# facebookresearch/pytorch3d

Measured on NVIDIA H100. Metric: rasterize frames/sec (fwd+bwd) 512^2 K=8, higher is better.
Workload: dtype f32

## Files before the change

pytorch3d_b200/csrc/binning.cuh:

```cuda
#pragma once
#include <climits>

#include "common.cuh"
#include "raster_math.cuh"

namespace b200r {

constexpr uint32_t RECT_EMPTY_X = 0x0000FFFFu;

__device__ __forceinline__ void pixel_range(float vmin, float vmax, int S, float range, int& lo, int& hi) {
  const float off = range * 0.5f, scale = (float)S / range, margin = 1e-3f + 1e-6f * (float)S;
  float a = (vmin + off) * scale - 0.5f - margin;
  float b = (vmax + off) * scale - 0.5f + margin;
  a = fminf(fmaxf(a, -1.0f), (float)S + 1.0f);
  b = fminf(fmaxf(b, -2.0f), (float)S);
  lo = max(0, (int)ceilf(a));
  hi = min(S - 1, (int)floorf(b));
}

__device__ __forceinline__ uint2 bbox_to_tile_rect(float xmin, float xmax, float ymin, float ymax, int H, int W,
                                                   float rx, float ry) {
  int ix_lo, ix_hi, iy_lo, iy_hi;
  pixel_range(xmin, xmax, W, rx, ix_lo, ix_hi);
  pixel_range(ymin, ymax, H, ry, iy_lo, iy_hi);
// ... 9 lines not shown
  const int64_t i = ((int64_t)blockIdx.x * 256 + threadIdx.x) * 4;
  pdl_trigger();
  if (i + 4 <= n && (reinterpret_cast<uintptr_t>(p) & 15u) == 0)
    *reinterpret_cast<int4*>(p + i) = make_int4(0, 0, 0, 0);
  else
    for (int64_t j = i; j < n && j < i + 4; ++j) p[j] = 0;
}

template <bool AGG = true>
__device__ __forceinline__ void warp_count_rect(uint2 r, int n, int TY, int TX, int* __restrict__ tile_count,
                                                int lane) {
  const bool empty = rect_empty(r);
  const int tx0 = r.x & 0xFFFF, tx1 = r.x >> 16, ty0 = r.y & 0xFFFF, ty1 = r.y >> 16;
  if (!AGG) {
    if (empty) return;
    for (int ty = ty0; ty <= ty1; ++ty)
      for (int tx = tx0; tx <= tx1; ++tx) atomicAdd(tile_count + (n * TY + ty) * TX + tx, 1);
    return;
  }
  const int w = empty ? 1 : tx1 - tx0 + 1;
  const int ntile = empty ? 0 : w * (ty1 - ty0 + 1);
  const int rounds = (int)__reduce_max_sync(0xffffffffu, (unsigned)ntile);
  int tx = tx0, ty = ty0;
  for (int i = 0; i < rounds; ++i) {
    const bool act = i < ntile;
    const int t = act ? (n * TY + ty) * TX + tx : -1 - lane;
    const int tprev = __shfl_up_sync(0xffffffffu, t, 1);
    const bool cont = act && lane > 0 && t == tprev;
    const unsigned conts = __ballot_sync(0xffffffffu, cont);
    if (act && !cont) {
      const unsigned after = lane == 31 ? 0u : conts >> (lane + 1);
      atomicAdd(tile_count + t, 1 + (__ffs((int)~after) - 1));
    }
    if (++tx > tx1) {
      tx = tx0;
      ++ty;
    }
  }
}

constexpr int ORDER_BITS = 21, ORDER_CLASSES = 3;
__device__ __forceinline__ int order_class(int count, int mean) { return count <= 0 ? 2 : (count > mean ? 0 : 1); }
__device__ __forceinline__ unsigned long long order_key(int count, int mean) {
  return 1ull << (ORDER_BITS * order_class(count, mean));
}

static __global__ void __launch_bounds__(1024) tile_scan_kernel(int* __restrict__ counts, int* __restrict__ offsets, int n,
                                                                int* __restrict__ order) {
  __shared__ long long warp_sums[32];
  __shared__ long long carry_s;
  __shared__ unsigned long long order_sums[32];
  __shared__ unsigned long long order_total, order_carry;
  __shared__ int nonempty_s;
  const int tid = threadIdx.x, lane = tid & 31, wid = tid >> 5;
  if (tid == 0) {
    carry_s = 0;
    nonempty_s = 0;
  }
  pdl_trigger();
  pdl_wait();
  __syncthreads();
  for (int base = 0; base < n; base += 8192) {
    const int i0 = base + tid * 8;
    int v[8];
    const bool vec = i0 + 8 <= n && ((reinterpret_cast<uintptr_t>(counts) | reinterpret_cast<uintptr_t>(offsets)) & 15u) == 0;
    if (vec) {
// ... 318 lines not shown
      } else {
        buf[phase * NT + i] = key;
        __syncthreads();
        other = buf[phase * NT + (i ^ d)];
        phase ^= 1;
      }
      B200R_CE64(other, (i & d) == 0);
    }
  }
#undef B200R_CE64
  return key;
}

template <int NT = TILE_THREADS>
__device__ __forceinline__ void cta_sort_segment(int* seg, int n, int* s_keys, int cap) {
  const bool in_smem = n <= cap;
  int* keys = in_smem ? s_keys : seg;
  if (in_smem)
    for (int i = threadIdx.x; i < n; i += NT) s_keys[i] = seg[i];
  __syncthreads();
  for (int k = 2; (k >> 1) < n; k <<= 1) {
    sort_sweep<true, NT>(keys, n, k);
    __syncthreads();
    for (int d = k >> 2; d > 0; d >>= 1) {
      sort_sweep<false, NT>(keys, n, d);
      __syncthreads();
    }
  }
  if (in_smem)
    for (int i = threadIdx.x; i < n; i += NT) seg[i] = s_keys[i];
  __syncthreads();
}

struct BinWorkspace {
  int* tile_count;
  int* tile_offset;
  int* tile_order;
  uint4* rect;
  int* pairs;
  int64_t capacity;
  size_t bytes;
};

inline int64_t default_pair_capacity(int64_t E, int N, int H, int W, int tile_h = TILE, int tile_w = TILE) {
  const int64_t tiles = (int64_t)div_up(H, tile_h) * div_up(W, tile_w);
  const int64_t exact = E * tiles;
  const int64_t heur = 32 * E + 64 * (int64_t)N * tiles;
  int64_t c = exact < heur ? exact : heur;
  if (c < 16) c = 16;
  if (c > 0x7fffffff) c = 0x7fffffff;
  return c;
}

inline BinWorkspace carve_workspace(void* base, int64_t E, int N, int H, int W, int64_t capacity, int tile_h = TILE,
                                    int tile_w = TILE) {
  BinWorkspace ws;
  const int64_t ntiles = (int64_t)N * div_up(H, tile_h) * div_up(W, tile_w);
  if (capacity <= 0) capacity = default_pair_capacity(E, N, H, W, tile_h, tile_w);
  ws.capacity = capacity;
  size_t off = 0;
  char* p = static_cast<char*>(base);
  ws.tile_count = reinterpret_cast<int*>(p + off);
  off = align_up(off + sizeof(int) * (size_t)ntiles, 16);
  ws.tile_offset = reinterpret_cast<int*>(p + off);
  off = align_up(off + sizeof(int) * (size_t)(ntiles + 1), 16);
  ws.tile_order = reinterpret_cast<int*>(p + off);
  off = align_up(off + sizeof(int) * (size_t)ntiles, 16);
  ws.rect = reinterpret_cast<uint4*>(p + off);
  off = align_up(off + sizeof(uint4) * (size_t)(E > 0 ? E : 1), 16);
  ws.pairs = reinterpret_cast<int*>(p + off);
  off = align_up(off + sizeof(int) * (size_t)capacity, 16);
  ws.bytes = off;
  return ws;
}

__device__ __forceinline__ unsigned box_pixel_mask(const float4 bx, const float (&col)[8], const float (&row)[4]) {
  unsigned xm = 0, ym = 0;
#pragma unroll
  for (int c = 0; c < 8; ++c) xm |= (!(col[c] > bx.y || col[c] < bx.x) ? 1u : 0u) << c;
#pragma unroll
  for (int r = 0; r < 4; ++r) ym |= (!(row[r] > bx.w || row[r] < bx.z) ? 1u : 0u) << (8 * r);
  return xm * ym;
}

__device__ __forceinline__ unsigned warp_transpose_bits(unsigned a, int lane) {
#pragma unroll
  for (int sft = 16; sft >= 1; sft >>= 1) {
    const unsigned lo = sft == 16 ? 0x0000FFFFu
                      : sft == 8 ? 0x00FF00FFu
                      : sft == 4 ? 0x0F0F0F0Fu
                      : sft == 2 ? 0x33333333u : 0x55555555u;
    const unsigned other = __shfl_xor_sync(0xffffffffu, a, sft);
    a = (lane & sft) ? ((a & ~lo) | ((other & ~lo) >> sft)) : ((a & lo) | ((other & lo) << sft));
  }
  return a;
}

}
```

pytorch3d_b200/csrc/raster_meshes.cu:

```cuda
#include <cfloat>
#include <climits>
#include <numeric>

#include "binning.cuh"
#include "bulk_copy.cuh"
#include "common.cuh"
#include "raster_math.cuh"

namespace b200r {

constexpr int SETUP_FACES = 256;
#ifndef B200R_MESH_TILE_H
#define B200R_MESH_TILE_H 16
#endif
constexpr int FTW = 16, FTH = B200R_MESH_TILE_H, FTHREADS = FTW * FTH;
static_assert(FTH == 16 || FTH == 8, "16x16 or 16x8 tiles");
constexpr int CHUNK = FTHREADS;
constexpr int SMEMQ_MAX_K = 32;

__device__ __forceinline__ bool face_is_drawable(const Face& f, bool cull_backfaces) {
  const float zmax = fmaxf(fmaxf(f.z0, f.z1), f.z2), zmin = fminf(fminf(f.z0, f.z1), f.z2);
  if (!(zmax >= 0.0f)) return false;
  if ((double)zmin < kEps) return false;
  const float area = edge_fn(f.x0, f.y0, f.x1, f.y1, f.x2, f.y2);
// ... 10 lines not shown
  ymax = fadd(fmaxf(fmaxf(f.y0, f.y1), f.y2), sqrt_blur);
}

constexpr size_t FACE_RECORD_BYTES = 4 * 16;

__device__ __forceinline__ void exact_pixel_range(float vmin, float vmax, int S, float range, int& lo, int& hi) {
  const float off = range * 0.5f, scale = (float)S / range, margin = 1e-3f + 1e-6f * (float)S;
  const float a = (vmin + off) * scale - 0.5f, b = (vmax + off) * scale - 0.5f;
  const float a0 = fminf(fmaxf(a - margin, -1.0f), (float)S + 1.0f), a1 = fminf(fmaxf(a + margin, -1.0f), (float)S + 1.0f);
  const float b0 = fminf(fmaxf(b + margin, -2.0f), (float)S), b1 = fminf(fmaxf(b - margin, -2.0f), (float)S);
  lo = max(0, (int)ceilf(a0));
  hi = min(S - 1, (int)floorf(b0));
  const bool lo_sure = lo == max(0, (int)ceilf(a1)) && a == a;
  const bool hi_sure = hi == min(S - 1, (int)floorf(b1)) && b == b;
  if (!lo_sure) {
    while (lo <= hi) {
      const float v = pix_to_ndc(lo, S, range);
      if (!(v > vmax || v < vmin)) break;
      ++lo;
    }
  }
  if (!hi_sure) {
    while (hi >= lo) {
      const float v = pix_to_ndc(hi, S, range);
      if (!(v > vmax || v < vmin)) break;
      --hi;
    }
  }
}

#ifndef B200R_SETUP_CTAS
#define B200R_SETUP_CTAS 1
#endif
template <bool INDEXED>
__global__ void __launch_bounds__(SETUP_FACES, B200R_SETUP_CTAS)
    mesh_setup_count_kernel(const float* __restrict__ face_verts, const float* __restrict__ verts, int64_t V,
                            const int64_t* __restrict__ faces, float* __restrict__ face_verts_out,
                            const int64_t* __restrict__ neighbor, int64_t F, const int64_t* __restrict__ first,
                            const int64_t* __restrict__ num, int N, int H, int W, int TY, int TX, float rx, float ry,
                            float sqrt_blur, int cull_backfaces, uint4* __restrict__ rect,
                            int* __restrict__ tile_count, float4* __restrict__ rec) {
  __shared__ __align__(16) float s_fv[SETUP_FACES * 9];
  __shared__ __align__(8) uint64_t bar;
  const int tid = threadIdx.x;
  const int64_t f0 = (int64_t)blockIdx.x * SETUP_FACES;
  const int nf = (int)min((int64_t)SETUP_FACES, F - f0);
  pdl_trigger();
  if (INDEXED) {
    for (int e = tid; e < nf * 3; e += SETUP_FACES) {
      const int64_t vi = __ldg(faces + f0 * 3 + e);
      const bool ok = vi >= 0 && vi < V;
      const float* v = verts + vi * 3;
      s_fv[e * 3 + 0] = ok ? __ldg(v + 0) : __int_as_float(0x7fc00000);
      s_fv[e * 3 + 1] = ok ? __ldg(v + 1) : __int_as_float(0x7fc00000);
      s_fv[e * 3 + 2] = ok ? __ldg(v + 2) : __int_as_float(0x7fc00000);
    }
    __syncthreads();
    for (int e = tid; e < nf * 9; e += SETUP_FACES) face_verts_out[f0 * 9 + e] = s_fv[e];
  } else {
    if (tid == 0) {
      mbar_init(&bar, 1);
      fence_mbar_init();
    }
    __syncthreads();
    cta_load_words(s_fv, face_verts + f0 * 9, nf * 9, &bar, 0);
  }
  uint2 r = make_uint2(RECT_EMPTY_X, 0u);
  int n = -1;
  const int64_t fi = f0 + tid;
  if (tid < nf) {
    const float* v = s_fv + tid * 9;
    const Face f = {v[0], v[1], v[2], v[3], v[4], v[5], v[6], v[7], v[8]};
    n = find_owner(first, num, N, fi);
    float4 box = make_float4(FLT_MAX, -FLT_MAX, FLT_MAX, -FLT_MAX);
    int4 rng = make_int4(1, 0, 1, 0);
    if (n >= 0 && face_is_drawable(f, cull_backfaces != 0)) {
      face_box(f, sqrt_blur, box.x, box.y, box.z, box.w);
      int ix_lo, ix_hi, iy_lo, iy_hi;
      exact_pixel_range(box.x, box.y, W, rx, ix_lo, ix_hi);
      exact_pixel_range(box.z, box.w, H, ry, iy_lo, iy_hi);
      if (ix_lo <= ix_hi && iy_lo <= iy_hi) {
        rng = make_int4(W - 1 - ix_hi, W - 1 - ix_lo, H - 1 - iy_hi, H - 1 - iy_lo);
        r = make_uint2((uint32_t)(rng.x / FTW) | ((uint32_t)(rng.y / FTW) << 16),
                       (uint32_t)(rng.z / FTH) | ((uint32_t)(rng.w / FTH) << 16));
      }
    }
    rect[fi] = make_uint4(r.x, r.y, (uint32_t)max(n, 0), 0u);
    const int nb = neighbor ? (int)__ldg(neighbor + fi) : -1;
    float4* out = rec + fi * 4;
    out[0] = make_float4(f.x0, f.y0, f.x1, f.y1);
    out[1] = make_float4(f.x2, f.y2, bary_denominator(f), __int_as_float((int)fi));
    out[2] = make_float4(f.z0, f.z1, f.z2, __int_as_float(nb));
    out[3] = sqrt_blur > 0.0f ? box
                              : make_float4(__int_as_float(rng.x), __int_as_float(rng.y), __int_as_float(rng.z),
                                            __int_as_float(rng.w));
  }
  pdl_wait();
  warp_count_rect(r, n, TY, TX, tile_count, tid & 31);
}

struct Hit {
  float z, dist, b0, b1, b2;
};

__device__ __forceinline__ void flag_tie();

template <bool WATCH>
__device__ __forceinline__ bool eval_pixel_face(float px, float py, const Face& f, float den, float blur_radius,
                                                bool persp, bool clip, bool full, float max_z, Hit& h) {
  const float e0 = edge_fn(px, py, f.x1, f.y1, f.x2, f.y2);
  const float e1 = edge_fn(px, py, f.x2, f.y2, f.x0, f.y0);
  const float e2 = edge_fn(px, py, f.x0, f.y0, f.x1, f.y1);
  float w0 = fdiv(e0, den), w1 = fdiv(e1, den), w2 = fdiv(e2, den);
  if (persp) bary_persp(w0, w1, w2, f.z0, f.z1, f.z2);
  float c0 = w0, c1 = w1, c2 = w2;
  if (clip) bary_clip(c0, c1, c2);
  const float pz = ffma(f.z2, c2, ffma(f.z0, c0, fmul(f.z1, c1)));
  if (!(pz >= 0.0f)) return false;
  if (full && !(pz < max_z)) {
    if (WATCH && pz == max_z) flag_tie();
    return false;
  }
  const bool inside = w0 > 0.0f && w1 > 0.0f && w2 > 0.0f;
  if (!inside && !(blur_radius > 0.0f)) return false;
  const float dist = point_tri_dist(px, py, f);
  if (!inside && dist >= blur_radius) return false;
  h.z = pz;
  h.dist = inside ? -dist : dist;
  h.b0 = c0;
  h.b1 = c1;
  h.b2 = c2;
// ... 205 lines not shown
};

__device__ __forceinline__ void stage_face(FaceChunk& s, int slot, const float* __restrict__ face_verts,
                                           const int64_t* __restrict__ neighbor, int f, float sqrt_blur,
                                           bool cull_backfaces) {
  const float* v = face_verts + (int64_t)f * 9;
  const Face fc = {__ldg(v + 0), __ldg(v + 1), __ldg(v + 2), __ldg(v + 3), __ldg(v + 4),
                   __ldg(v + 5), __ldg(v + 6), __ldg(v + 7), __ldg(v + 8)};
  float xmin = FLT_MAX, xmax = -FLT_MAX, ymin = FLT_MAX, ymax = -FLT_MAX;
  if (face_is_drawable(fc, cull_backfaces)) face_box(fc, sqrt_blur, xmin, xmax, ymin, ymax);
  s.box[slot] = make_float4(xmin, xmax, ymin, ymax);
  s.a[slot] = make_float4(fc.x0, fc.y0, fc.x1, fc.y1);
  s.b[slot] = make_float4(fc.x2, fc.y2, bary_denominator(fc), __int_as_float(f));
  const int nb = neighbor ? (int)__ldg(neighbor + f) : -1;
  s.c[slot] = make_float4(fc.z0, fc.z1, fc.z2, __int_as_float(nb));
}

template <typename T>
__device__ __forceinline__ void out_store(T* ptr, const T v) {
  __stcs(ptr, v);
}

struct FineParams {
  const float* face_verts;
  const int64_t* neighbor;
  const float4* rec;
  const int64_t* first;
  const int64_t* num;
  const int* tile_offset;
  const int* tile_order;
  int row_stride;
  int* pairs;
  int64_t capacity;
  int n0;
  int N, H, W, K, TY, TX;
  float rx, ry, blur_radius, sqrt_blur;
  int persp, clip, cull;
  int smem_ints;
  int64_t* pix_to_face;
  float* zbuf;
  float* bary;
  float* dists;
};

__device__ __forceinline__ void thread_pixel(int tile_x, int tile_y, int& xo, int& yo) {
  const int lane = threadIdx.x & 31, w = threadIdx.x >> 5;
  xo = tile_x * TILE + (w & 1) * 8 + (lane & 7);
  yo = tile_y * TILE + (w >> 1) * 4 + (lane >> 3);
}
__device__ __forceinline__ void fthread_pixel(int tile_x, int tile_y, int& xo, int& yo) {
  const int lane = threadIdx.x & 31, w = threadIdx.x >> 5;
  xo = tile_x * FTW + (w & 1) * 8 + (lane & 7);
  yo = tile_y * FTH + (w >> 1) * 4 + (lane >> 3);
}

__device__ __forceinline__ float warp_min(float v) {
#pragma unroll
  for (int d = 16; d > 0; d >>= 1) v = fminf(v, __shfl_xor_sync(0xffffffffu, v, d));
  return v;
}
__device__ __forceinline__ float warp_max(float v) {
#pragma unroll
  for (int d = 16; d > 0; d >>= 1) v = fmaxf(v, __shfl_xor_sync(0xffffffffu, v, d));
  return v;
}

// ... 138 lines not shown
  if (NB && nb != -1 && q.offer_neighbor(h, fi, nb)) return;
  q.offer(h, fi);
}

__device__ __forceinline__ float face_depth_lower_bound(const float4 fa, const float4 fb, const float4 fc, float cx,
                                                        float cy, float hx, float hy, bool persp, bool clip) {
  const float z0 = fc.x, z1 = fc.y, z2 = fc.z;
  if (clip) return fminf(fminf(z0, z1), z2) * (1.0f - 1e-6f);
  if (persp) return -FLT_MAX;
  const float x0 = fa.x, y0 = fa.y, x1 = fa.z, y1 = fa.w, x2 = fb.x, y2 = fb.y;
  const float rd = 1.0f / fabsf(fb.z);
  const float e0 = (cx - x1) * (y2 - y1) - (cy - y1) * (x2 - x1);
  const float e1 = (cx - x2) * (y0 - y2) - (cy - y2) * (x0 - x2);
  const float e2 = (cx - x0) * (y1 - y0) - (cy - y0) * (x1 - x0);
  const float num = z0 * e0 + z1 * e1 + z2 * e2;
  const float gxn = z0 * (y2 - y1) + z1 * (y0 - y2) + z2 * (y1 - y0);
  const float gyn = z0 * (x2 - x1) + z1 * (x0 - x2) + z2 * (x1 - x0);
  const float pzc = (fb.z < 0.0f ? -num : num) * rd;
  const float spread = (fabsf(gxn) * hx + fabsf(gyn) * hy) * rd;
  const float dx = fmaxf(fmaxf(fabsf(cx - x0), fabsf(cx - x1)), fabsf(cx - x2)) + hx;
  const float dy = fmaxf(fmaxf(fabsf(cy - y0), fabsf(cy - y1)), fabsf(cy - y2)) + hy;
  const float lx = fmaxf(fmaxf(x0, x1), x2) - fminf(fminf(x0, x1), x2);
  const float ly = fmaxf(fmaxf(y0, y1), y2) - fminf(fminf(y0, y1), y2);
  const float zabs = fmaxf(fmaxf(fabsf(z0), fabsf(z1)), fabsf(z2));
  const float margin = 1e-5f * (zabs * (dx * ly + dy * lx) * rd + fabsf(pzc) + spread);
  const float lb = pzc - spread - margin;
  return lb == lb ? lb : -FLT_MAX;
}

enum { ORDER_ARRIVAL = 0, ORDER_INDEX = 1 };

template <class Q, bool NB, bool SCAN>
__device__ __forceinline__ void fine_tile_body(const FineParams& p, FineStage& sh, Q& q, int tile_x, int tile_y, int n,
                                               int seg_begin, int count, bool overflow, int order, bool valid, int lc,
                                               int lr) {
  const int tid = threadIdx.x, lane = tid & 31;
  const bool persp = p.persp != 0, clip = p.clip != 0;
  const float blur_radius = p.blur_radius;
  const bool sorted_walk = order == ORDER_INDEX;
  const bool sort_staged = sorted_walk && !overflow && count <= CHUNK;
  if (sorted_walk && !overflow && count > CHUNK)
    cta_sort_segment<FTHREADS>(p.pairs + seg_begin, count, reinterpret_cast<int*>(&sh), p.smem_ints);
  if (tid < FTW + FTH) {
    if (tid < FTW)
      sh.col[tid] = pix_to_ndc(p.W - 1 - (tile_x * FTW + tid), p.W, p.rx);
    else
      sh.row[tid - FTW] = pix_to_ndc(p.H - 1 - (tile_y * FTH + tid - FTW), p.H, p.ry);
  }
  if (!sorted_walk && tid == FTW + FTH) sh.tie = 0;

  for (int base = 0; base < count; base += CHUNK) {
    const int nc = min(CHUNK, count - base);
    const int nwords = (nc + 31) >> 5;
    if (base > 0) __syncthreads();
    int f = INT_MAX;
    if (tid < nc) f = overflow ? (int)(p.first[n] + base + tid) : p.pairs[seg_begin + base + tid];
    if (sort_staged) {
      f = cta_sort256<FTHREADS>(f, nc, sh.u.sort_buf);
      if (nc > 32) __syncthreads();
    }
    if (tid < nc) {
      const float4* r = p.rec + (int64_t)f * 4;
      const float4 ra = __ldg(r + 0), rb = __ldg(r + 1), rc = __ldg(r + 2), rd = __ldg(r + 3);
      sh.a[tid] = ra;
      sh.b[tid] = rb;
      sh.c[tid] = rc;
      if (SCAN) {
        const int gx = __float_as_int(rd.x), gy = __float_as_int(rd.y), gz = __float_as_int(rd.z),
                  gw = __float_as_int(rd.w);
        const int c_lo = max(gx - tile_x * FTW, 0), c_hi = min(gy - tile_x * FTW, FTW - 1);
        const int r_lo = max(gz - tile_y * FTH, 0), r_hi = min(gw - tile_y * FTH, FTH - 1);
        sh.rng[tid] = (c_lo > c_hi || r_lo > r_hi) ? 1u
                                                   : (unsigned)(c_lo | (c_hi << 8) | (r_lo << 16) | (r_hi << 24));
      } else {
        sh.u.box[tid] = rd;
      }
    }
    if (SCAN) {
      for (int w = 0; w < nwords; ++w) sh.u.mask[w][tid] = 0u;
    }
    __syncthreads();
    if (SCAN) {
#ifndef B200R_SCAN_LANES
#define B200R_SCAN_LANES 4
#endif
      constexpr int SL = B200R_SCAN_LANES;
      const int dr = tid & (SL - 1);
      for (int fslot = tid / SL; fslot < nc; fslot += FTHREADS / SL) {
        const unsigned rg = sh.rng[fslot];
// ... 83 lines not shown
            __all_sync(0xffffffffu, !keep1 || (cmin >= b1.x && cmax <= b1.y && rmin >= b1.z && rmax <= b1.w));
        if (all0 && all1) {
          m0 = __ballot_sync(0xffffffffu, keep0);
          m1 = __ballot_sync(0xffffffffu, keep1);
        } else {
          float col[8], row[4];
#pragma unroll
          for (int c = 0; c < 8; ++c) col[c] = sh.col[(lc & 8) + c];
#pragma unroll
          for (int r = 0; r < 4; ++r) row[r] = sh.row[(lr & 12) + r];
          if (keep0) m0 = box_pixel_mask(b0, col, row);
          if (keep1) m1 = box_pixel_mask(b1, col, row);
          m0 = warp_transpose_bits(m0, lane);
          if (sub + 32 < nc) m1 = warp_transpose_bits(m1, lane);
        }
      }
      unsigned long long mine = valid ? (((unsigned long long)m1 << 32) | m0) : 0ull;
      while (__any_sync(0xffffffffu, mine != 0ull)) {
        if (mine != 0ull) {
          const int j = sub + __ffsll((long long)mine) - 1;
          mine &= mine - 1ull;
          consider_face<Q, NB>(sh, j, px, py, blur_radius, persp, clip, q);
        }
      }
    }
  }
}

__device__ __forceinline__ bool tile_saw_tie(const FineStage& sh) {
  return __syncthreads_or(sh.tie) != 0;
}

struct TileWork {
  int tile_x, tile_y, n, seg_begin, count;
  bool overflow;
};
__device__ __forceinline__ TileWork tile_work(const FineParams& p) {
  pdl_wait();
  TileWork t;
  int i;
  if (p.tile_order != nullptr) {
    i = p.tile_order[((p.n0 + blockIdx.z) * p.TY + blockIdx.y) * p.TX + blockIdx.x];
    t.tile_x = i % p.TX;
    const int r = i / p.TX;
    t.tile_y = r % p.TY;
    t.n = r / p.TY;
  } else {
    t.tile_x = blockIdx.x;
    t.tile_y = (int)((blockIdx.y * (unsigned)p.row_stride) % (unsigned)p.TY);
    t.n = p.n0 + blockIdx.z;
    i = (t.n * p.TY + t.tile_y) * p.TX + t.tile_x;
  }
  t.seg_begin = p.tile_offset[i];
  const int seg_end = p.tile_offset[i + 1];
  t.overflow = (int64_t)seg_end > p.capacity || seg_end == INT_MAX;
  t.count = t.overflow ? (int)p.num[t.n] : seg_end - t.seg_begin;
  return t;
}

template <bool NB, bool SCAN>
__device__ __forceinline__ int first_walk_order(const TileWork& t) {
  if (t.overflow || NB) return ORDER_INDEX;
  if (SCAN) return ORDER_ARRIVAL;
  return ORDER_INDEX;
}

#ifndef B200R_FINE_CTAS
#define B200R_FINE_CTAS 4
#endif
#ifndef B200R_FINE_SCAN_CTAS
#define B200R_FINE_SCAN_CTAS 3
#endif
#ifndef B200R_SMEMQ_CTAS
#define B200R_SMEMQ_CTAS 3
#endif
#ifndef B200R_SMEMQ_SCAN_CTAS
#define B200R_SMEMQ_SCAN_CTAS 2
#endif

template <int KMAX, bool NB, bool SCAN>
__global__ void __launch_bounds__(FTHREADS, SCAN ? B200R_FINE_SCAN_CTAS : B200R_FINE_CTAS) mesh_fine_kernel(const FineParams p) {
  extern __shared__ __align__(16) unsigned char smem_raw[];
  FineStage& sh = *reinterpret_cast<FineStage*>(smem_raw);
  const int tid = threadIdx.x, lane = tid & 31;
  const TileWork t = tile_work(p);
  const int tile_x = t.tile_x, tile_y = t.tile_y, n = t.n;
  if (t.count == 0) {
    write_empty_tile<KMAX>(p, n, tile_x, tile_y);
    return;
  }
  int xo, yo;
  fthread_pixel(tile_x, tile_y, xo, yo);
  const bool valid = xo < p.W && yo < p.H;
  const int lc = xo - tile_x * FTW, lr = yo - tile_y * FTH;

  RegQueue<KMAX> rq;
  rq.q.init();
  rq.pay = reinterpret_cast<float4*>(smem_raw + sizeof(FineStage)) + tid;
  rq.K = p.K;
  TopK<KMAX>& q = rq.q;
  float4* pay = rq.pay;
  const int K = p.K;
  int order = first_walk_order<NB, SCAN>(t);
  for (;;) {
  fine_tile_body<RegQueue<KMAX>, NB, SCAN>(p, sh, rq, tile_x, tile_y, n, t.seg_begin, t.count, t.overflow, order, valid,
                                           lc, lr);
  bool stored = false;
  int slot[KMAX];
  q.sort(slot);
  const int64_t o = (((int64_t)n * p.H + yo) * p.W + xo) * K;
  if constexpr ((KMAX % 4) == 0) {
   if (K == KMAX) {
    const int odd = lane & 1;
    const bool vA = __shfl_sync(0xffffffffu, (int)valid, lane & ~1) != 0;
    const bool vB = __shfl_sync(0xffffffffu, (int)valid, lane | 1) != 0;
    const int64_t oa = o - (int64_t)odd * KMAX;
    store_pair_pieces<KMAX / 2>(reinterpret_cast<float4*>(p.pix_to_face + oa), [&](int i) {
      const long long i0 = 2 * i >= q.size ? -1ll : (long long)q.id[2 * i];
      const long long i1 = 2 * i + 1 >= q.size ? -1ll : (long long)q.id[2 * i + 1];
      return make_float4(__int_as_float((int)(i0 & 0xffffffffll)), __int_as_float((int)(i0 >> 32)),
                         __int_as_float((int)(i1 & 0xffffffffll)), __int_as_float((int)(i1 >> 32)));
    }, odd, vA, vB);
    store_pair_pieces<KMAX / 4>(reinterpret_cast<float4*>(p.zbuf + oa), [&](int i) {
      const int k0 = 4 * i;
      return make_float4(k0 + 0 >= q.size ? -1.0f : q.z[k0 + 0], k0 + 1 >= q.size ? -1.0f : q.z[k0 + 1],
                         k0 + 2 >= q.size ? -1.0f : q.z[k0 + 2], k0 + 3 >= q.size ? -1.0f : q.z[k0 + 3]);
    }, odd, vA, vB);
    store_pair_pieces<KMAX / 4>(reinterpret_cast<float4*>(p.dists + oa), [&](int i) {
      float d[4];
#pragma unroll
      for (int u = 0; u < 4; ++u) d[u] = 4 * i + u >= q.size ? -1.0f : pay[slot[4 * i + u] * FTHREADS].x;
      return make_float4(d[0], d[1], d[2], d[3]);
    }, odd, vA, vB);
    store_pair_pieces<3 * KMAX / 4>(reinterpret_cast<float4*>(p.bary + oa * 3), [&](int i) {
      const int k0 = 4 * (i / 3), c = i % 3;
      float4 w[2];
#pragma unroll
      for (int u = 0; u < 2; ++u) {
// ... 9 lines not shown
  if (!stored && valid) {
#pragma unroll
    for (int k = 0; k < KMAX; ++k) {
      if (k < K) {
        const bool e = k >= q.size;
        const float4 w = e ? make_float4(-1.f, -1.f, -1.f, -1.f) : pay[slot[k] * FTHREADS];
        p.pix_to_face[o + k] = e ? -1ll : (long long)q.id[k];
        p.zbuf[o + k] = e ? -1.0f : q.z[k];
        p.dists[o + k] = w.x;
        p.bary[(o + k) * 3 + 0] = w.y;
        p.bary[(o + k) * 3 + 1] = w.z;
        p.bary[(o + k) * 3 + 2] = w.w;
      }
    }
  }
  if (order != ORDER_ARRIVAL || !tile_saw_tie(sh)) return;
  order = ORDER_INDEX;
  rq.reset();
  }
}

__device__ __forceinline__ void recompute_hit(const FineParams& p, int fi, float px, float py, Hit& h) {
  const float4* r = p.rec + (int64_t)fi * 4;
  const float4 fa = __ldg(r + 0), fb = __ldg(r + 1), fc = __ldg(r + 2);
  const Face f = {fa.x, fa.y, fc.x, fa.z, fa.w, fc.y, fb.x, fb.y, fc.z};
  eval_pixel_face<false>(px, py, f, fb.z, p.blur_radius, p.persp != 0, p.clip != 0, false, 0.0f, h);
}

template <bool NB, bool SCAN>
__global__ void __launch_bounds__(FTHREADS, SCAN ? B200R_SMEMQ_SCAN_CTAS : B200R_SMEMQ_CTAS) mesh_fine_smemq_kernel(const FineParams p) {
  extern __shared__ __align__(16) unsigned char smem_raw[];
  FineStage& sh = *reinterpret_cast<FineStage*>(smem_raw);
  const int tid = threadIdx.x, lane = tid & 31;
  const TileWork t = tile_work(p);
  const int tile_x = t.tile_x, tile_y = t.tile_y, n = t.n;
  if (t.count == 0) {
    write_empty_tile<0>(p, n, tile_x, tile_y);
    return;
  }
  int xo, yo;
  fthread_pixel(tile_x, tile_y, xo, yo);
  const bool valid = xo < p.W && yo < p.H;
  const int lc = xo - tile_x * FTW, lr = yo - tile_y * FTH;
  const int K = p.K;

  SmemQueue<NB> q;
  q.init(smem_raw + sizeof(FineStage), K, tid);
  int order = first_walk_order<NB, SCAN>(t);
  for (;;) {
  fine_tile_body<SmemQueue<NB>, NB, SCAN>(p, sh, q, tile_x, tile_y, n, t.seg_begin, t.count, t.overflow, order, valid,
                                          lc, lr);
  q.sort();
  const float px = sh.col[lc], py = sh.row[lr];
  const int64_t o = (((int64_t)n * p.H + yo) * p.W + xo) * K;
  if ((K & 7) == 0) {
    const int odd = lane & 1;
    const bool vA = __shfl_sync(0xffffffffu, (int)valid, lane & ~1) != 0;
    const bool vB = __shfl_sync(0xffffffffu, (int)valid, lane | 1) != 0;
    const int64_t oa = o - (int64_t)odd * K, ob = oa + K;
    for (int g = 0; g < K; g += 8) {
      float4 pi[4], pzv[2], pd[2], pb[6];
      float z[8], d[8], b[24];
      int id[8];
#pragma unroll
      for (int u = 0; u < 8; ++u) {
        Hit h = {-1.0f, -1.0f, -1.0f, -1.0f, -1.0f};
        id[u] = -1;
        if (g + u < q.size) {
          id[u] = q.qi[(g + u) * FTHREADS];
          recompute_hit(p, id[u], px, py, h);
        }
        z[u] = h.z;
        d[u] = h.dist;
        b[3 * u + 0] = h.b0;
        b[3 * u + 1] = h.b1;
        b[3 * u + 2] = h.b2;
      }
#pragma unroll
      for (int u = 0; u < 4; ++u)
        pi[u] = make_float4(__int_as_float(id[2 * u]), __int_as_float(id[2 * u] >> 31),
                            __int_as_float(id[2 * u + 1]), __int_as_float(id[2 * u + 1] >> 31));
#pragma unroll
      for (int u = 0; u < 2; ++u) {
// ... 386 lines not shown
      float g[9] = {0.f, 0.f, 0.f, 0.f, 0.f, 0.f, 0.f, 0.f, 0.f};
      if (face >= 0) {
        const int64_t i = o + k0 + j;
        const float gz = __ldg(p.grad_zbuf + i);
        const float gd = __ldg(p.grad_dists + i);
        const float gb0 = __ldg(p.grad_bary + i * 3);
        const float gb1 = __ldg(p.grad_bary + i * 3 + 1);
        const float gb2 = __ldg(p.grad_bary + i * 3 + 2);
        backward_one(p, px, py, face, gz, gd, gb0, gb1, gb2, persp, clip, g);
      }
      warp_scatter(p, face, g, lane);
    }
  }
}

}

__global__ void __launch_bounds__(256) mesh_gather_kernel(const float* __restrict__ verts, int64_t V,
                                                          const int64_t* __restrict__ faces, int64_t F,
                                                          float* __restrict__ face_verts_out) {
  const int64_t e = (int64_t)blockIdx.x * blockDim.x + threadIdx.x;
  if (e >= F * 3) return;
  const int64_t vi = __ldg(faces + e);
  const bool ok = vi >= 0 && vi < V;
#pragma unroll
  for (int c = 0; c < 3; ++c) face_verts_out[e * 3 + c] = ok ? __ldg(verts + vi * 3 + c) : __int_as_float(0x7fc00000);
}

using namespace b200r;

extern "C" size_t b200r_rasterize_meshes_workspace_bytes(int64_t F, int32_t N, int32_t H, int32_t W,
                                                         int64_t pair_capacity) {
  if (F < 0 || N < 0 || H < 0 || W < 0) return 0;
  return carve_workspace(nullptr, F, N, H, W, pair_capacity, FTH, FTW).bytes +
         FACE_RECORD_BYTES * (size_t)(F > 0 ? F : 1);
}

static int forward_impl(const float* face_verts, const float* verts, int64_t V, const int64_t* faces,
                        float* face_verts_out, int64_t F, const int64_t* first, const int64_t* num,
                        const int64_t* neighbor, int32_t N, int32_t H, int32_t W, float blur_radius, int32_t K,
                        int32_t perspective_correct, int32_t clip_barycentric_coords, int32_t cull_backfaces,
                        int64_t* pix_to_face, float* zbuf, float* bary, float* dists, void* workspace,
                        size_t workspace_bytes, int64_t pair_capacity, void* stream_) {
  cudaStream_t stream = static_cast<cudaStream_t>(stream_);
  if (K > B200R_MAX_K) return fail(B200R_ERR_INVALID_ARGUMENT, "Must have points_per_pixel <= 150");
  if (F < 0 || N < 0 || H < 0 || W < 0 || K < 0) return fail(B200R_ERR_INVALID_ARGUMENT, "negative size");
  if (F > INT_MAX) return fail(B200R_ERR_INVALID_ARGUMENT, "more than 2^31-1 packed faces are not supported");
  if ((int64_t)N * H * W * K == 0) return B200R_OK;
  const int TY = div_up(H, FTH), TX = div_up(W, FTW);
  if (TY > 0xFFFE || TX > 0xFFFE) return fail(B200R_ERR_INVALID_ARGUMENT, "image too large");
  const int64_t ntiles = (int64_t)N * TY * TX;
  if (ntiles > INT_MAX) return fail(B200R_ERR_INVALID_ARGUMENT, "too many tiles");
  BinWorkspace ws = carve_workspace(workspace, F, N, H, W, pair_capacity, FTH, FTW);
  const size_t nrec = (size_t)(F > 0 ? F : 1);
  if (workspace == nullptr || workspace_bytes < ws.bytes + FACE_RECORD_BYTES * nrec)
    return fail(B200R_ERR_WORKSPACE, "workspace too small for rasterize_meshes_forward");
  float4* rec = reinterpret_cast<float4*>(static_cast<char*>(workspace) + ws.bytes);

  const float rx = ndc_range(W, H), ry = ndc_range(H, W);
  const float sqrt_blur = sqrtf(blur_radius);

  const bool prof = profiling_enabled();
  if (prof) phase_timer().record(0, stream);
  zero_ints_kernel<<<(unsigned)((ntiles + 1023) / 1024), 256, 0, stream>>>(ws.tile_count, ntiles);
  B200R_LAUNCHED("zero_ints_kernel");
  if (F > 0) {
    const unsigned sgrid = (unsigned)((F + SETUP_FACES - 1) / SETUP_FACES);
#define B200R_SETUP_LAUNCH(KERNEL, ...) B200R_CUDA_OK(launch_chained(KERNEL, dim3(sgrid), dim3(SETUP_FACES), 0, stream, __VA_ARGS__))
    if (faces != nullptr) {
      B200R_SETUP_LAUNCH(mesh_setup_count_kernel<true>, (const float*)nullptr, verts, V, faces, face_verts_out, neighbor, F,
                         first, num, N, H, W, TY, TX, rx, ry, sqrt_blur, cull_backfaces, ws.rect, ws.tile_count, rec);
      face_verts = face_verts_out;
    } else {
      B200R_SETUP_LAUNCH(mesh_setup_count_kernel<false>, face_verts, (const float*)nullptr, (int64_t)0,
                         (const int64_t*)nullptr, (float*)nullptr, neighbor, F, first, num, N, H, W, TY, TX, rx, ry,
                         sqrt_blur, cull_backfaces, ws.rect, ws.tile_count, rec);
    }
#undef B200R_SETUP_LAUNCH
    B200R_LAUNCHED("mesh_setup_count_kernel");
  }
  int* const tile_order = (blur_radius > 0.0f && ntiles < (1ll << ORDER_BITS)) ? ws.tile_order : nullptr;
  B200R_CUDA_OK(launch_chained(tile_scan_kernel, dim3(1), dim3(1024), 0, stream, ws.tile_count, ws.tile_offset,
                               (int)ntiles, tile_order));
  B200R_LAUNCHED("tile_scan_kernel");
  if (F > 0) {
    B200R_CUDA_OK(launch_chained(tile_fill_kernel<true>, dim3((unsigned)((F + 255) / 256)), dim3(256), 0, stream,
                                 ws.rect, F, TY, TX, ws.tile_count, ws.pairs, ws.capacity));
    B200R_LAUNCHED("tile_fill_kernel");
  }
  if (prof) phase_timer().record(1, stream);
  FineParams p;
  p.face_verts = face_verts;
  p.neighbor = neighbor;
  p.rec = rec;
  p.n0 = 0;
  p.first = first;
  p.num = num;
  p.tile_offset = ws.tile_offset;
  p.tile_order = tile_order;
  p.row_stride = 1;
  if (!(blur_radius > 0.0f)) {
    p.row_stride = (int)(TY * 0.382) | 1;
    while (std::gcd(p.row_stride, TY) != 1) p.row_stride += 2;
  }
  p.pairs = ws.pairs;
  p.capacity = ws.capacity;
  p.N = N; p.H = H; p.W = W; p.K = K; p.TY = TY; p.TX = TX;
  p.rx = rx; p.ry = ry; p.blur_radius = blur_radius; p.sqrt_blur = sqrt_blur;
  p.persp = perspective_correct; p.clip = clip_barycentric_coords; p.cull = cull_backfaces;
  p.smem_ints = 0;
  p.pix_to_face = pix_to_face; p.zbuf = zbuf; p.bary = bary; p.dists = dists;
  const unsigned grid = (unsigned)ntiles;
  const bool no_blur = !(blur_radius > 0.0f);
  int dev_ = 0;
  B200R_CUDA_OK(cudaGetDevice(&dev_));
#define B200R_FINE_LAUNCH(KERNEL, SMEM_MAX, SMEM)                                                         \
  do {                                                                                                   \
    static bool configured[64] = {};                                                                     \
    if (dev_ < 0 || dev_ >= 64 || !configured[dev_]) {                                                   \
      B200R_CUDA_OK(cudaFuncSetAttribute(KERNEL, cudaFuncAttributeMaxDynamicSharedMemorySize, (int)(SMEM_MAX))); \
      if (dev_ >= 0 && dev_ < 64) configured[dev_] = true;                                               \
    }                                                                                                    \
    p.smem_ints = (int)((SMEM) / sizeof(int));                                                           \
    for (p.n0 = 0; p.n0 < N; p.n0 += 65535) {                                                            \
      const dim3 grid3((unsigned)TX, (unsigned)TY, (unsigned)min(N - p.n0, 65535));                      \
      B200R_CUDA_OK(launch_chained(KERNEL, grid3, dim3(FTHREADS), (SMEM), stream, p));                   \
    }                                                                                                    \
  } while (0)
#define B200R_FINE(KM)                                                                                    \
  do {                                                                                                   \
    constexpr size_t smem_ = sizeof(FineStage) + sizeof(float4) * KM * FTHREADS;                         \
    if (neighbor && no_blur)                                                                             \
      B200R_FINE_LAUNCH((mesh_fine_kernel<KM, true, true>), smem_, smem_);                               \
    else if (neighbor)                                                                                   \
      B200R_FINE_LAUNCH((mesh_fine_kernel<KM, true, false>), smem_, smem_);                              \
    else if (no_blur)                                                                                    \
      B200R_FINE_LAUNCH((mesh_fine_kernel<KM, false, true>), smem_, smem_);                              \
    else                                                                                                 \
      B200R_FINE_LAUNCH((mesh_fine_kernel<KM, false, false>), smem_, smem_);                             \
// ... 142 lines not shown
```

Before: 19170.

## Bin faces into per-tile chunked append lists instead of count-scan-fill

For the no-blur path with K up to 32, the setup kernel now appends face ids directly into per-tile lists. Each list is a fixed 256-entry chunk plus 1024-entry chunks taken from a shared pool through atomics. This removes the single-CTA prefix-scan kernel and the separate tile_fill pass that re-walks every face rectangle. In exchange it adds atomics and warp shuffles during setup, chunk-table indirection when the fine kernel reads ids, and an overflow fallback when the pool runs out.

```diff
diff --git a/pytorch3d_b200/csrc/binning.cuh b/pytorch3d_b200/csrc/binning.cuh
--- a/pytorch3d_b200/csrc/binning.cuh
+++ b/pytorch3d_b200/csrc/binning.cuh
@@ -65,6 +65,96 @@
       const unsigned after = lane == 31 ? 0u : conts >> (lane + 1);
       atomicAdd(tile_count + t, 1 + (__ffs((int)~after) - 1));
     }
+    if (++tx > tx1) {
+      tx = tx0;
+      ++ty;
+    }
+  }
+}
+
+constexpr int LIST_CHUNK = 256;
+constexpr int POOL_CHUNK = 1024;
+constexpr int LIST_TABLE = 31;
+constexpr unsigned LIST_MAX = LIST_CHUNK + (unsigned)POOL_CHUNK * LIST_TABLE;
+constexpr unsigned LIST_OVERFLOW = 1u << 30;
+
+struct TileLists {
+  int* count;
+  int* chunk;
+  unsigned long long* pool_used;
+  int* ids;
+  int64_t ntiles, pool_chunks;
+};
+
+__device__ __forceinline__ int list_chunk(unsigned pos) {
+  return pos < LIST_CHUNK ? 0 : (int)((pos - LIST_CHUNK) / POOL_CHUNK) + 1;
+}
+__device__ __forceinline__ unsigned list_chunk_start(int k) {
+  return k == 0 ? 0u : LIST_CHUNK + (unsigned)POOL_CHUNK * (k - 1);
+}
+__device__ __forceinline__ unsigned list_take_ahead(int k) { return k == 0 ? LIST_CHUNK / 2 : list_chunk_start(k); }
+
+__device__ __forceinline__ int64_t list_chunk_base(const TileLists& L, int64_t tile, int k) {
+  if (k == 0) return tile * LIST_CHUNK;
+  const int e = __ldg(L.chunk + tile * LIST_TABLE + (k - 1));
+  return L.ntiles * LIST_CHUNK + (int64_t)(e - 1) * POOL_CHUNK - (int64_t)list_chunk_start(k);
+}
+
+__device__ __forceinline__ int64_t list_take_chunk(const TileLists& L, int64_t tile, int k, bool needs) {
+  int* entry = L.chunk + tile * LIST_TABLE + (k - 1);
+  int e = *reinterpret_cast<volatile int*>(entry);
+  if (e == 0) {
+    const unsigned long long b = atomicAdd(L.pool_used, 1ull);
+    if (b >= (unsigned long long)L.pool_chunks) {
+      if (needs) atomicOr(L.count + tile, (int)LIST_OVERFLOW);
+      return -1;
+    }
+    const int old = atomicCAS(entry, 0, (int)b + 1);
+    e = old == 0 ? (int)b + 1 : old;
+  }
+  return L.ntiles * LIST_CHUNK + (int64_t)(e - 1) * POOL_CHUNK - (int64_t)list_chunk_start(k);
+}
+
+__device__ __forceinline__ void st_list_entry(int* p, int v) {
+  asm volatile(
+      "{\n\t.reg .b64 pol;\n\tcreatepolicy.fractional.L2::evict_last.b64 pol, 1.0;\n\t"
+      "st.global.L2::cache_hint.b32 [%0], %1, pol;\n\t}" ::"l"(p), "r"(v)
+      : "memory");
+}
+
+__device__ __forceinline__ void warp_append_rect(uint2 r, int n, int TY, int TX, int e, const TileLists& L, int lane) {
+  const bool empty = rect_empty(r);
+  const int tx0 = r.x & 0xFFFF, tx1 = r.x >> 16, ty0 = r.y & 0xFFFF, ty1 = r.y >> 16;
+  const int w = empty ? 1 : tx1 - tx0 + 1;
+  const int ntile = empty ? 0 : w * (ty1 - ty0 + 1);
+  const int rounds = (int)__reduce_max_sync(0xffffffffu, (unsigned)ntile);
+  const unsigned at_or_below = 0xffffffffu >> (31 - lane);
+  int tx = tx0, ty = ty0;
+  for (int i = 0; i < rounds; ++i) {
+    const bool act = i < ntile;
+    const int t = act ? (n * TY + ty) * TX + tx : -1 - lane;
+    const int tprev = __shfl_up_sync(0xffffffffu, t, 1);
+    const bool cont = act && lane > 0 && t == tprev;
+    const unsigned conts = __ballot_sync(0xffffffffu, cont);
+    const unsigned heads = __ballot_sync(0xffffffffu, act && !cont);
+    const int leader = act ? 31 - __clz((int)(heads & at_or_below)) : lane;
+    unsigned base = 0;
+    if (act && !cont) {
+      const unsigned after = lane == 31 ? 0u : conts >> (lane + 1);
+      base = atomicAdd(reinterpret_cast<unsigned*>(L.count) + t, (unsigned)__ffs((int)~after));
+    }
+    const unsigned pos = __shfl_sync(0xffffffffu, base, leader) + (unsigned)(lane - leader);
+    const int k = list_chunk(pos);
+    const bool pooled = act && k >= 1 && k <= LIST_TABLE;
+    const bool finder = pooled && (lane == leader || pos == list_chunk_start(k));
+    long long cb = (long long)t * LIST_CHUNK;
+    if (finder) cb = list_take_chunk(L, t, k, true);
+    const unsigned finders = __ballot_sync(0xffffffffu, finder);
+    const int src = pooled ? 31 - __clz((int)(finders & at_or_below)) : lane;
+    const long long got = __shfl_sync(0xffffffffu, cb, src);
+    if (pooled) cb = got;
+    if (act && k <= LIST_TABLE && cb >= 0) st_list_entry(L.ids + cb + pos, e);
+    if (act && k < LIST_TABLE && pos == list_take_ahead(k)) list_take_chunk(L, t, k + 1, false);
     if (++tx > tx1) {
       tx = tx0;
       ++ty;
@@ -449,6 +539,51 @@
   __syncthreads();
 }
 
+template <int NT, class Key>
+__device__ __forceinline__ void cta_sort_keys(Key key, int n) {
+  for (int k = 2; (k >> 1) < n; k <<= 1) {
+    for (int d = k, mirror = 1; d > 0; d = mirror ? k >> 2 : d >> 1, mirror = 0) {
+      for (int i = threadIdx.x; i < n; i += NT) {
+        const int j = mirror ? (i ^ (d - 1)) : (i ^ d);
+        if (j > i && j < n) {
+          int& ki = key(i);
+          int& kj = key(j);
+          const int a = ki, b = kj;
+          if (b < a) {
+            ki = b;
+            kj = a;
+          }
+        }
+      }
+      __syncthreads();
+    }
+  }
+}
+
+template <int NT>
+__device__ __forceinline__ void cta_sort_list(const TileLists& L, int64_t tile, int n, int* s_keys, int cap) {
+  const bool in_smem = n <= cap;
+  if (in_smem) {
+    for (int k = 0, at = 0; at < n; at = (int)list_chunk_start(++k)) {
+      const int64_t b = list_chunk_base(L, tile, k);
+      const int end = min(n, (int)list_chunk_start(k + 1));
+      for (int i = at + threadIdx.x; i < end; i += NT) s_keys[i] = L.ids[b + i];
+    }
+  }
+  __syncthreads();
+  cta_sort_keys<NT>([&](int i) -> int& {
+    return in_smem ? s_keys[i] : L.ids[list_chunk_base(L, tile, list_chunk((unsigned)i)) + i];
+  }, n);
+  if (in_smem) {
+    for (int k = 0, at = 0; at < n; at = (int)list_chunk_start(++k)) {
+      const int64_t b = list_chunk_base(L, tile, k);
+      const int end = min(n, (int)list_chunk_start(k + 1));
+      for (int i = at + threadIdx.x; i < end; i += NT) L.ids[b + i] = s_keys[i];
+    }
+  }
+  __syncthreads();
+}
+
 struct BinWorkspace {
   int* tile_count;
   int* tile_offset;
@@ -491,6 +626,39 @@
   return ws;
 }
 
+struct ListWorkspace {
+  TileLists lists;
+  int* tile_order;
+  int64_t zero_ints;
+  size_t bytes;
+};
+
+inline ListWorkspace carve_list_workspace(void* base, int64_t E, int N, int H, int W, int64_t capacity, int tile_h,
+                                          int tile_w) {
+  ListWorkspace ws;
+  const int64_t ntiles = (int64_t)N * div_up(H, tile_h) * div_up(W, tile_w);
+  if (capacity <= 0) capacity = default_pair_capacity(E, N, H, W, tile_h, tile_w);
+  int64_t pool_chunks = (capacity - ntiles * LIST_CHUNK) / POOL_CHUNK;
+  pool_chunks = pool_chunks < 0 ? 0 : (pool_chunks > (1 << 30) ? (1 << 30) : pool_chunks);
+  ws.lists.ntiles = ntiles;
+  ws.lists.pool_chunks = pool_chunks;
+  size_t off = 0;
+  char* p = static_cast<char*>(base);
+  ws.lists.count = reinterpret_cast<int*>(p + off);
+  off = align_up(off + sizeof(int) * (size_t)ntiles, 16);
+  ws.lists.chunk = reinterpret_cast<int*>(p + off);
+  off = align_up(off + sizeof(int) * (size_t)ntiles * LIST_TABLE, 16);
+  ws.lists.pool_used = reinterpret_cast<unsigned long long*>(p + off);
+  off = align_up(off + sizeof(unsigned long long), 16);
+  ws.zero_ints = (int64_t)(off / sizeof(int));
+  ws.tile_order = reinterpret_cast<int*>(p + off);
+  off = align_up(off + sizeof(int) * (size_t)ntiles, 16);
+  ws.lists.ids = reinterpret_cast<int*>(p + off);
+  off = align_up(off + sizeof(int) * ((size_t)ntiles * LIST_CHUNK + (size_t)pool_chunks * POOL_CHUNK), 16);
+  ws.bytes = off;
+  return ws;
+}
+
 __device__ __forceinline__ unsigned box_pixel_mask(const float4 bx, const float (&col)[8], const float (&row)[4]) {
   unsigned xm = 0, ym = 0;
 #pragma unroll
diff --git a/pytorch3d_b200/csrc/raster_meshes.cu b/pytorch3d_b200/csrc/raster_meshes.cu
--- a/pytorch3d_b200/csrc/raster_meshes.cu
+++ b/pytorch3d_b200/csrc/raster_meshes.cu
@@ -66,14 +66,14 @@
 #ifndef B200R_SETUP_CTAS
 #define B200R_SETUP_CTAS 1
 #endif
-template <bool INDEXED>
+template <bool INDEXED, bool LISTS>
 __global__ void __launch_bounds__(SETUP_FACES, B200R_SETUP_CTAS)
     mesh_setup_count_kernel(const float* __restrict__ face_verts, const float* __restrict__ verts, int64_t V,
                             const int64_t* __restrict__ faces, float* __restrict__ face_verts_out,
                             const int64_t* __restrict__ neighbor, int64_t F, const int64_t* __restrict__ first,
                             const int64_t* __restrict__ num, int N, int H, int W, int TY, int TX, float rx, float ry,
                             float sqrt_blur, int cull_backfaces, uint4* __restrict__ rect,
-                            int* __restrict__ tile_count, float4* __restrict__ rec) {
+                            int* __restrict__ tile_count, const TileLists lists, float4* __restrict__ rec) {
   __shared__ __align__(16) float s_fv[SETUP_FACES * 9];
   __shared__ __align__(8) uint64_t bar;
   const int tid = threadIdx.x;
@@ -119,7 +119,7 @@
                        (uint32_t)(rng.z / FTH) | ((uint32_t)(rng.w / FTH) << 16));
       }
     }
-    rect[fi] = make_uint4(r.x, r.y, (uint32_t)max(n, 0), 0u);
+    if (!LISTS) rect[fi] = make_uint4(r.x, r.y, (uint32_t)max(n, 0), 0u);
     const int nb = neighbor ? (int)__ldg(neighbor + fi) : -1;
     float4* out = rec + fi * 4;
     out[0] = make_float4(f.x0, f.y0, f.x1, f.y1);
@@ -130,7 +130,10 @@
                                             __int_as_float(rng.w));
   }
   pdl_wait();
-  warp_count_rect(r, n, TY, TX, tile_count, tid & 31);
+  if (LISTS)
+    warp_append_rect(r, n, TY, TX, (int)fi, lists, tid & 31);
+  else
+    warp_count_rect(r, n, TY, TX, tile_count, tid & 31);
 }
 
 struct Hit {
@@ -402,6 +405,7 @@
   int row_stride;
   int* pairs;
   int64_t capacity;
+  TileLists lists;
   int n0;
   int N, H, W, K, TY, TX;
   float rx, ry, blur_radius, sqrt_blur;
@@ -606,15 +610,19 @@
 
 template <class Q, bool NB, bool SCAN>
 __device__ __forceinline__ void fine_tile_body(const FineParams& p, FineStage& sh, Q& q, int tile_x, int tile_y, int n,
-                                               int seg_begin, int count, bool overflow, int order, bool valid, int lc,
+                                               int seg, int count, bool overflow, int order, bool valid, int lc,
                                                int lr) {
   const int tid = threadIdx.x, lane = tid & 31;
   const bool persp = p.persp != 0, clip = p.clip != 0;
   const float blur_radius = p.blur_radius;
   const bool sorted_walk = order == ORDER_INDEX;
   const bool sort_staged = sorted_walk && !overflow && count <= CHUNK;
-  if (sorted_walk && !overflow && count > CHUNK)
-    cta_sort_segment<FTHREADS>(p.pairs + seg_begin, count, reinterpret_cast<int*>(&sh), p.smem_ints);
+  if (sorted_walk && !overflow && count > CHUNK) {
+    if (SCAN)
+      cta_sort_list<FTHREADS>(p.lists, seg, count, reinterpret_cast<int*>(&sh), p.smem_ints);
+    else
+      cta_sort_segment<FTHREADS>(p.pairs + seg, count, reinterpret_cast<int*>(&sh), p.smem_ints);
+  }
   if (tid < FTW + FTH) {
     if (tid < FTW)
       sh.col[tid] = pix_to_ndc(p.W - 1 - (tile_x * FTW + tid), p.W, p.rx);
@@ -628,7 +636,10 @@
     const int nwords = (nc + 31) >> 5;
     if (base > 0) __syncthreads();
     int f = INT_MAX;
-    if (tid < nc) f = overflow ? (int)(p.first[n] + base + tid) : p.pairs[seg_begin + base + tid];
+    if (tid < nc)
+      f = overflow ? (int)(p.first[n] + base + tid)
+          : SCAN   ? p.lists.ids[list_chunk_base(p.lists, seg, list_chunk((unsigned)base)) + base + tid]
+                   : p.pairs[seg + base + tid];
     if (sort_staged) {
       f = cta_sort256<FTHREADS>(f, nc, sh.u.sort_buf);
       if (nc > 32) __syncthreads();
@@ -778,9 +789,10 @@
 }
 
 struct TileWork {
-  int tile_x, tile_y, n, seg_begin, count;
+  int tile_x, tile_y, n, seg, count;
   bool overflow;
 };
+template <bool SCAN>
 __device__ __forceinline__ TileWork tile_work(const FineParams& p) {
   pdl_wait();
   TileWork t;
@@ -797,10 +809,17 @@
     t.n = p.n0 + blockIdx.z;
     i = (t.n * p.TY + t.tile_y) * p.TX + t.tile_x;
   }
-  t.seg_begin = p.tile_offset[i];
+  if (SCAN) {
+    t.seg = i;
+    const unsigned c = (unsigned)p.lists.count[i];
+    t.overflow = c > LIST_MAX;
+    t.count = t.overflow ? (int)p.num[t.n] : (int)c;
+    return t;
+  }
+  t.seg = p.tile_offset[i];
   const int seg_end = p.tile_offset[i + 1];
   t.overflow = (int64_t)seg_end > p.capacity || seg_end == INT_MAX;
-  t.count = t.overflow ? (int)p.num[t.n] : seg_end - t.seg_begin;
+  t.count = t.overflow ? (int)p.num[t.n] : seg_end - t.seg;
   return t;
 }
 
@@ -829,7 +848,7 @@
   extern __shared__ __align__(16) unsigned char smem_raw[];
   FineStage& sh = *reinterpret_cast<FineStage*>(smem_raw);
   const int tid = threadIdx.x, lane = tid & 31;
-  const TileWork t = tile_work(p);
+  const TileWork t = tile_work<SCAN>(p);
   const int tile_x = t.tile_x, tile_y = t.tile_y, n = t.n;
   if (t.count == 0) {
     write_empty_tile<KMAX>(p, n, tile_x, tile_y);
@@ -849,7 +868,7 @@
   const int K = p.K;
   int order = first_walk_order<NB, SCAN>(t);
   for (;;) {
-  fine_tile_body<RegQueue<KMAX>, NB, SCAN>(p, sh, rq, tile_x, tile_y, n, t.seg_begin, t.count, t.overflow, order, valid,
+  fine_tile_body<RegQueue<KMAX>, NB, SCAN>(p, sh, rq, tile_x, tile_y, n, t.seg, t.count, t.overflow, order, valid,
                                            lc, lr);
   bool stored = false;
   int slot[KMAX];
@@ -925,7 +944,7 @@
   extern __shared__ __align__(16) unsigned char smem_raw[];
   FineStage& sh = *reinterpret_cast<FineStage*>(smem_raw);
   const int tid = threadIdx.x, lane = tid & 31;
-  const TileWork t = tile_work(p);
+  const TileWork t = tile_work<SCAN>(p);
   const int tile_x = t.tile_x, tile_y = t.tile_y, n = t.n;
   if (t.count == 0) {
     write_empty_tile<0>(p, n, tile_x, tile_y);
@@ -941,7 +960,7 @@
   q.init(smem_raw + sizeof(FineStage), K, tid);
   int order = first_walk_order<NB, SCAN>(t);
   for (;;) {
-  fine_tile_body<SmemQueue<NB>, NB, SCAN>(p, sh, q, tile_x, tile_y, n, t.seg_begin, t.count, t.overflow, order, valid,
+  fine_tile_body<SmemQueue<NB>, NB, SCAN>(p, sh, q, tile_x, tile_y, n, t.seg, t.count, t.overflow, order, valid,
                                           lc, lr);
   q.sort();
   const float px = sh.col[lc], py = sh.row[lr];
@@ -1394,8 +1413,9 @@
 extern "C" size_t b200r_rasterize_meshes_workspace_bytes(int64_t F, int32_t N, int32_t H, int32_t W,
                                                          int64_t pair_capacity) {
   if (F < 0 || N < 0 || H < 0 || W < 0) return 0;
-  return carve_workspace(nullptr, F, N, H, W, pair_capacity, FTH, FTW).bytes +
-         FACE_RECORD_BYTES * (size_t)(F > 0 ? F : 1);
+  const size_t compact = carve_workspace(nullptr, F, N, H, W, pair_capacity, FTH, FTW).bytes;
+  const size_t lists = carve_list_workspace(nullptr, F, N, H, W, pair_capacity, FTH, FTW).bytes;
+  return (compact > lists ? compact : lists) + FACE_RECORD_BYTES * (size_t)(F > 0 ? F : 1);
 }
 
 static int forward_impl(const float* face_verts, const float* verts, int64_t V, const int64_t* faces,
@@ -1413,39 +1433,49 @@
   if (TY > 0xFFFE || TX > 0xFFFE) return fail(B200R_ERR_INVALID_ARGUMENT, "image too large");
   const int64_t ntiles = (int64_t)N * TY * TX;
   if (ntiles > INT_MAX) return fail(B200R_ERR_INVALID_ARGUMENT, "too many tiles");
-  BinWorkspace ws = carve_workspace(workspace, F, N, H, W, pair_capacity, FTH, FTW);
+  const BinWorkspace ws = carve_workspace(workspace, F, N, H, W, pair_capacity, FTH, FTW);
+  const ListWorkspace lws = carve_list_workspace(workspace, F, N, H, W, pair_capacity, FTH, FTW);
+  const size_t bin_bytes = ws.bytes > lws.bytes ? ws.bytes : lws.bytes;
   const size_t nrec = (size_t)(F > 0 ? F : 1);
-  if (workspace == nullptr || workspace_bytes < ws.bytes + FACE_RECORD_BYTES * nrec)
+  if (workspace == nullptr || workspace_bytes < bin_bytes + FACE_RECORD_BYTES * nrec)
     return fail(B200R_ERR_WORKSPACE, "workspace too small for rasterize_meshes_forward");
-  float4* rec = reinterpret_cast<float4*>(static_cast<char*>(workspace) + ws.bytes);
+  float4* rec = reinterpret_cast<float4*>(static_cast<char*>(workspace) + bin_bytes);
+  const bool use_lists = !(blur_radius > 0.0f) && K <= SMEMQ_MAX_K;
 
   const float rx = ndc_range(W, H), ry = ndc_range(H, W);
   const float sqrt_blur = sqrtf(blur_radius);
 
   const bool prof = profiling_enabled();
   if (prof) phase_timer().record(0, stream);
-  zero_ints_kernel<<<(unsigned)((ntiles + 1023) / 1024), 256, 0, stream>>>(ws.tile_count, ntiles);
+  if (use_lists)
+    zero_ints_kernel<<<(unsigned)((lws.zero_ints + 1023) / 1024), 256, 0, stream>>>(lws.lists.count, lws.zero_ints);
+  else
+    zero_ints_kernel<<<(unsigned)((ntiles + 1023) / 1024), 256, 0, stream>>>(ws.tile_count, ntiles);
   B200R_LAUNCHED("zero_ints_kernel");
   if (F > 0) {
     const unsigned sgrid = (unsigned)((F + SETUP_FACES - 1) / SETUP_FACES);
 #define B200R_SETUP_LAUNCH(KERNEL, ...) B200R_CUDA_OK(launch_chained(KERNEL, dim3(sgrid), dim3(SETUP_FACES), 0, stream, __VA_ARGS__))
     if (faces != nullptr) {
-      B200R_SETUP_LAUNCH(mesh_setup_count_kernel<true>, (const float*)nullptr, verts, V, faces, face_verts_out, neighbor, F,
-                         first, num, N, H, W, TY, TX, rx, ry, sqrt_blur, cull_backfaces, ws.rect, ws.tile_count, rec);
+      B200R_SETUP_LAUNCH((use_lists ? mesh_setup_count_kernel<true, true> : mesh_setup_count_kernel<true, false>),
+                         (const float*)nullptr, verts, V, faces, face_verts_out, neighbor, F, first, num, N, H, W, TY,
+                         TX, rx, ry, sqrt_blur, cull_backfaces, ws.rect, ws.tile_count, lws.lists, rec);
       face_verts = face_verts_out;
     } else {
-      B200R_SETUP_LAUNCH(mesh_setup_count_kernel<false>, face_verts, (const float*)nullptr, (int64_t)0,
-                         (const int64_t*)nullptr, (float*)nullptr, neighbor, F, first, num, N, H, W, TY, TX, rx, ry,
-                         sqrt_blur, cull_backfaces, ws.rect, ws.tile_count, rec);
+      B200R_SETUP_LAUNCH((use_lists ? mesh_setup_count_kernel<false, true> : mesh_setup_count_kernel<false, false>),
+                         face_verts, (const float*)nullptr, (int64_t)0, (const int64_t*)nullptr, (float*)nullptr,
+                         neighbor, F, first, num, N, H, W, TY, TX, rx, ry, sqrt_blur, cull_backfaces, ws.rect,
+                         ws.tile_count, lws.lists, rec);
     }
 #undef B200R_SETUP_LAUNCH
     B200R_LAUNCHED("mesh_setup_count_kernel");
   }
   int* const tile_order = (blur_radius > 0.0f && ntiles < (1ll << ORDER_BITS)) ? ws.tile_order : nullptr;
-  B200R_CUDA_OK(launch_chained(tile_scan_kernel, dim3(1), dim3(1024), 0, stream, ws.tile_count, ws.tile_offset,
-                               (int)ntiles, tile_order));
-  B200R_LAUNCHED("tile_scan_kernel");
-  if (F > 0) {
+  if (!use_lists) {
+    B200R_CUDA_OK(launch_chained(tile_scan_kernel, dim3(1), dim3(1024), 0, stream, ws.tile_count, ws.tile_offset,
+                                 (int)ntiles, tile_order));
+    B200R_LAUNCHED("tile_scan_kernel");
+  }
+  if (F > 0 && !use_lists) {
     B200R_CUDA_OK(launch_chained(tile_fill_kernel<true>, dim3((unsigned)((F + 255) / 256)), dim3(256), 0, stream,
                                  ws.rect, F, TY, TX, ws.tile_count, ws.pairs, ws.capacity));
     B200R_LAUNCHED("tile_fill_kernel");
@@ -1467,6 +1497,7 @@
   }
   p.pairs = ws.pairs;
   p.capacity = ws.capacity;
+  p.lists = lws.lists;
   p.N = N; p.H = H; p.W = W; p.K = K; p.TY = TY; p.TX = TX;
   p.rx = rx; p.ry = ry; p.blur_radius = blur_radius; p.sqrt_blur = sqrt_blur;
   p.persp = perspective_correct; p.clip = clip_barycentric_coords; p.cull = cull_backfaces;
```

Result: faster. 19720, median of 6 (+2.9%).
